# KdaiP/StableTTS

Hardware: NVIDIA H100
Metric: mel-frames/sec through CFM DiT estimator (ODE solve, all evaluations) (higher is better)
Workload: dtype f32 (split-bf16x3 tensor-core operands; FFN convs fp16 activations x fp16 hi/lo weights, 2 passes; fp32 accumulate)

## Files before the change

### stabletts_b200/csrc/gemm_epilogue.cuh

```cuda
#pragma once
#include "common.cuh"
#include <type_traits>
#include "tc_ptx.cuh"

namespace st {

enum : int { EM_PLAIN = 0, EM_SILU = 1, EM_GELU = 2, EM_ROPE = 3, EM_LN = 4, EM_RESID = 5,
             EM_SILU_OUT = 6,
             EM_MISH = 7 };

struct TcParams {
    int n_src, Cs0, Cs1, taps, dil, N, a_bmod, BB, T;
    int m_tiles_per_b, n_tiles, total_tiles;
    int flags, B, film_H, c_clamp, resid_clamp, rope_H;
    long film_bstride, gate_bstride;
    const float *bias, *mask, *film, *gate, *resid, *rope_cs;
    int mode;
    float* out_f32; bf16* out_hi; bf16* out_lo;
    int out16, u16;
    int ln_mask_out;
    const float *ln_shift, *ln_scale, *film2;
    float* out2_f32; bf16* u_hi; bf16* u_lo;
    long ada_bstride, film2_bstride;
    int ksplit, split_bb;
// ... 66 lines not shown

__device__ __forceinline__ float2 lds2_volatile(uint32_t a) {
    float2 v;
    asm volatile("ld.volatile.shared.v2.f32 {%0, %1}, [%2];" : "=f"(v.x), "=f"(v.y) : "r"(a));
    return v;
}

__device__ __forceinline__ void named_bar_sync(int id) { asm volatile("bar.sync %0, 128;" ::"r"(id) : "memory"); }

template <typename T>
__device__ __forceinline__ T* row_ptr(T* base, long off) {
    T* r;
    asm volatile("add.s64 %0, %1, %2;" : "=l"(r) : "l"(base), "l"(off * (long)sizeof(T)));
    return r;
}

__device__ __forceinline__ void st2_if(float* a, float x, float y, bool on) {
    asm volatile("{\n\t.reg .pred q;\n\tsetp.ne.b32 q, %3, 0;\n\t@q st.global.v2.f32 [%0], {%1, %2};\n\t}"
                 ::"l"(a), "f"(x), "f"(y), "r"((int)on));
}
__device__ __forceinline__ void st1_if(bf16* a, uint32_t v, bool on) {
    asm volatile("{\n\t.reg .pred q;\n\tsetp.ne.b32 q, %2, 0;\n\t@q st.global.b32 [%0], %1;\n\t}" ::"l"(a), "r"(v), "r"((int)on));
}

}

enum : int { EV_BIAS = 0, EV_FILM_G, EV_FILM_B, EV_GATE, EV_FILM2_G, EV_FILM2_B, EV_LN_SHIFT, EV_LN_SCALE, EV_COUNT };
constexpr int EPI_VEC_BYTES = EV_COUNT * 256 * 4;

template <int BN, int MODE>
__device__ __forceinline__ void stage_epi_vectors(const TcParams& p, int bb, int n0, uint32_t vs, int bar_id) {
    static_assert(BN == 256, "one column pair per thread of the warpgroup");
    epi::named_bar_sync(bar_id);
    const int c = 2 * (threadIdx.x & 127);
    const int mb = bb % p.B, cb = min(bb, p.c_clamp);
    auto put = [&](int v, const float* src) {
        const float2 x = epi::ld2(src + c);
        asm volatile("st.shared.v2.f32 [%0], {%1, %2};" ::"r"(vs + (v * BN + c) * 4), "f"(x.x), "f"(x.y) : "memory");
    };
    if (p.flags & EPI_BIAS) put(EV_BIAS, p.bias + n0);
    if (MODE != EM_ROPE) {
        if (p.flags & EPI_FILM) {
            const float* film = p.film + (long)mb * p.film_bstride + n0;
            put(EV_FILM_G, film); put(EV_FILM_B, film + p.film_H);
        }
        if (p.flags & EPI_GATE) put(EV_GATE, p.gate + (long)cb * p.gate_bstride + n0);
    }
    if (MODE == EM_LN) {
        const long ab = (long)cb * p.ada_bstride;
        put(EV_LN_SHIFT, p.ln_shift + ab); put(EV_LN_SCALE, p.ln_scale + ab);
        if (p.film2) {
            const float* film2 = p.film2 + (long)mb * p.film2_bstride;
            put(EV_FILM2_G, film2); put(EV_FILM2_B, film2 + p.film_H);
        }
    }
}

template <int MODE>
__device__ __forceinline__ void epilogue_wide(const TcParams& p, int bb, int t0, int n0, float (&acc)[128], uint32_t vs,
                                              int bar_id) {
    using namespace epi;
    constexpr int BN = 256, NJ = BN / 8;
    named_bar_sync(bar_id);
    constexpr bool ROPE = MODE == EM_ROPE, LN = MODE == EM_LN, SO = MODE == EM_SILU_OUT;
    constexpr bool RES = MODE == EM_RESID || MODE == EM_LN || SO;
    const int lane = threadIdx.x & 31, w = (threadIdx.x >> 5) & 3;
    const int cq = 2 * (lane & 3);
    const int mb = bb % p.B;
    const int f = p.flags;
    const bool bias = f & EPI_BIAS, film = f & EPI_FILM, gate = f & EPI_GATE;
    const bool plain = ROPE || (f & (EPI_FILM | EPI_MASK | EPI_GATE | EPI_RESID)) == 0;
    const bool has_resid = RES && (f & EPI_RESID);
    const float rfill = plain || (f & (EPI_FILM | EPI_MASK | EPI_GATE | EPI_RESID)) == EPI_MASK ? -0.f : 0.f;
    const bool f16 = p.out16 != 0, has_film2 = LN && p.film2;
    const bool has_2 = p.out2_f32 && (SO || has_film2);
    const int rope_rot = 2 * p.rope_H - n0, rope_q = p.rope_H - n0;
    constexpr int RD = 8;
    enum : int { FMT_ANY, FMT_F16, FMT_SPLIT };

#pragma unroll
    for (int r = 0; r < 2; ++r) {
        const int t = t0 + 16 * w + (lane >> 2) + 8 * r;
        const bool row_ok = t < p.T;
        const int tcl = min(t, p.T - 1);
        const float mrow = (!ROPE && p.mask) ? __ldg(p.mask + (long)mb * p.T + tcl) : 1.f;
        const float m = (f & EPI_MASK) ? mrow : 1.f;
        const long orow = ((long)bb * p.T + tcl) * p.N + n0 + cq;
        float4 cs4[2];
        if constexpr (ROPE) {
            const float* cs = p.rope_cs + (long)tcl * 32;
            cs4[0] = __ldg(reinterpret_cast<const float4*>(cs + 2 * cq));
            cs4[1] = __ldg(reinterpret_cast<const float4*>(cs + 2 * (8 + cq)));
        }
        const bool st_f32 = row_ok && p.out_f32, st_f16 = row_ok && p.out_hi && f16, st_split = row_ok && p.out_hi && !f16;
        const bool st_2 = row_ok && has_2;
        float* const of = row_ptr(p.out_f32, orow);
        float* const o2 = SO || LN ? row_ptr(p.out2_f32, orow) : nullptr;
        bf16* const oh = row_ptr(p.out_hi, orow);
        bf16* const ol = row_ptr(p.out_lo, orow);
        const float* const rs = RES ? row_ptr(p.resid, ((long)min(bb, p.resid_clamp) * p.T + tcl) * p.N + n0 + cq) : nullptr;
        uint32_t vsr;
        asm volatile("mov.b32 %0, %1;" : "=r"(vsr) : "r"(vs + cq * 4));
        auto vec = [&](int v, int j) { return lds2(vsr + (v * BN + 8 * j) * 4); };
        float s1 = 0.f;

        auto row = [&](auto fmt) {
            float2 ring[RD];
            if constexpr (RES) {
#pragma unroll
                for (int j = 0; j < RD; ++j) ring[j] = ld2_ring(rs + 8 * j, has_resid, rfill);
            }
#pragma unroll
            for (int j = 0; j < NJ; ++j) {
                const int i = (j / 16) * 64 + (j % 16) * 4 + 2 * r;
                float x0 = acc[i], x1 = acc[i + 1];
                float2 rr;
                if constexpr (RES) {
                    rr = ring[j % RD];
                    if (j + RD < NJ) ring[j % RD] = ld2_ring(rs + 8 * (j + RD), has_resid, rfill);
                }
                if constexpr (ROPE) {
                    const int jj = j % 8, hh = j / 8;
                    const bool rot = 64 * hh < rope_rot;
                    if (jj == 0 && rot) {
#pragma unroll
                        for (int k = 0; k < 2; ++k) {
                            const int ia = ((j + k) / 16) * 64 + ((j + k) % 16) * 4 + 2 * r;
                            const int i2 = ((j + k + 2) / 16) * 64 + ((j + k + 2) % 16) * 4 + 2 * r;
                            float u0 = acc[ia], u1 = acc[ia + 1], y0 = acc[i2], y1 = acc[i2 + 1];
                            if (bias) { const float2 b = vec(EV_BIAS, j + k); u0 += b.x; u1 += b.y; }
                            if (bias) { const float2 b = vec(EV_BIAS, j + k + 2); y0 += b.x; y1 += b.y; }
                            const float4 c4 = cs4[k];
                            acc[ia] = u0 * c4.x - y0 * c4.y; acc[ia + 1] = u1 * c4.z - y1 * c4.w;
                            acc[i2] = y0 * c4.x + u0 * c4.y; acc[i2 + 1] = y1 * c4.z + u1 * c4.w;
                        }
                    }
                    x0 = acc[i]; x1 = acc[i + 1];
                    if (bias && !(jj < 4 && rot)) { const float2 b = vec(EV_BIAS, j); x0 += b.x; x1 += b.y; }
                    if (64 * hh < rope_q) { x0 *= kQScale; x1 *= kQScale; }
                } else {
                    float &a0 = acc[i], &a1 = acc[i + 1];
                    if (bias) { const float2 b = vec(EV_BIAS, j); a0 += b.x; a1 += b.y; }
                    if constexpr (MODE == EM_SILU) { a0 = silu_fast(a0); a1 = silu_fast(a1); }
                    if constexpr (MODE == EM_GELU) { a0 = gelu_f(a0); a1 = gelu_f(a1); }
                    if (film) {
                        const float2 fg = vec(EV_FILM_G, j), fb = vec(EV_FILM_B, j);
                        a0 = fmaf(fg.x, a0, fb.x); a1 = fmaf(fg.y, a1, fb.y);
                    }
                    float g0 = m, g1 = m;
                    if (gate) { const float2 g2 = vec(EV_GATE, j); g0 *= g2.x; g1 *= g2.y; }
                    if constexpr (RES) {
                        a0 = fmaf(a0, g0, rr.x); a1 = fmaf(a1, g1, rr.y);
                    } else if (!plain) {
                        a0 *= g0; a1 *= g1;
                    }
                    x0 = a0; x1 = a1;
                }
                st2_if(of + 8 * j, x0, x1, st_f32);
                float h0 = x0, h1 = x1;
                if constexpr (SO) { h0 = silu_fast(x0); h1 = silu_fast(x1); st2_if(o2 + 8 * j, h0, h1, st_2); }
                if constexpr (decltype(fmt)::value != FMT_SPLIT) st1_if(oh + 8 * j, pack_f16x2_sat(h0, h1), st_f16);
                if constexpr (decltype(fmt)::value != FMT_F16) {
                    uint32_t hw, lw;
                    split_bf16x2(h0, h1, hw, lw);
                    st1_if(oh + 8 * j, hw, st_split); st1_if(ol + 8 * j, lw, st_split);
                }
                if constexpr (LN) {
                    if (has_film2) {
                        const float2 fg = vec(EV_FILM2_G, j), fb = vec(EV_FILM2_B, j);
                        x0 = (fg.x * x0 + fb.x) * mrow; x1 = (fg.y * x1 + fb.y) * mrow;
                    }
                    st2_if(o2 + 8 * j, x0, x1, st_2);
                    acc[i] = x0; acc[i + 1] = x1;
                    s1 += x0 + x1;
                }
            }
        };
        if constexpr (RES) {
            row(std::integral_constant<int, FMT_ANY>());
        } else if (f16) {
// ... 22 lines not shown
                const float2 s4 = lds2_volatile(vsr + (EV_LN_SHIFT * BN + 8 * j) * 4);
                const float2 c4 = lds2_volatile(vsr + (EV_LN_SCALE * BN + 8 * j) * 4);
                u0 = ((acc[i] - mean) * rstd * (1.f + c4.x) + s4.x) * mo;
                u1 = ((acc[i + 1] - mean) * rstd * (1.f + c4.y) + s4.y) * mo;
            };
            if (p.u16) {
#pragma unroll
                for (int j = 0; j < NJ; ++j) {
                    float u0, u1;
                    u_pair(j, u0, u1);
                    st1_if(uh + 8 * j, pack_f16x2_sat(u0, u1), row_ok);
                }
            } else {
#pragma unroll
                for (int j = 0; j < NJ; ++j) {
                    float u0, u1;
                    uint32_t hw, lw;
                    u_pair(j, u0, u1);
                    split_bf16x2(u0, u1, hw, lw);
                    st1_if(uh + 8 * j, hw, row_ok); st1_if(ul + 8 * j, lw, row_ok);
                }
            }
        }
    }
}

template <int BN, int MODE>
__device__ __forceinline__ void epilogue_narrow(const TcParams& p, int bb, int t0, int n0, float (&acc)[BN / 2]) {
    using namespace epi;
    constexpr bool ROPE = MODE == EM_ROPE, SO = MODE == EM_SILU_OUT;
    constexpr bool RES = MODE == EM_RESID || SO;
    static_assert(BN <= 128 && MODE != EM_LN, "the fused LayerNorm runs on full-row 256-channel tiles (epilogue_wide)");
    constexpr int NJ = BN / 8;
    const int lane = threadIdx.x & 31, w = (threadIdx.x >> 5) & 3;
    const int cq = 2 * (lane & 3);
    const int mb = bb % p.B;
    const bool plain = ROPE || (p.flags & (EPI_FILM | EPI_MASK | EPI_GATE | EPI_RESID)) == 0;
    const bool mask_only = !ROPE && (p.flags & (EPI_FILM | EPI_MASK | EPI_GATE | EPI_RESID)) == EPI_MASK;
    const bool has_resid = RES && (p.flags & EPI_RESID);
    const float* film = p.film + (long)mb * p.film_bstride;
    const float* gate = p.gate + (long)min(bb, p.c_clamp) * p.gate_bstride;

    constexpr int RD = 8;

#pragma unroll
    for (int r = 0; r < 2; ++r) {
// ... 93 lines not shown
```

### stabletts_b200/csrc/gemm_tc.cu

```cuda
#include "common.cuh"
#include "gemm_epilogue.cuh"
#include <cuda.h>
#include <cudaTypedefs.h>
#include <mutex>
#include <unordered_map>
#include <string>
#include <cstring>
#include <cstdlib>

namespace st {

static_assert(ST_TEST_MODE_PLAIN == EM_PLAIN && ST_TEST_MODE_SILU == EM_SILU && ST_TEST_MODE_GELU == EM_GELU &&
              ST_TEST_MODE_ROPE == EM_ROPE && ST_TEST_MODE_LN == EM_LN && ST_TEST_MODE_RESID == EM_RESID &&
              ST_TEST_MODE_SILU_OUT == EM_SILU_OUT && ST_TEST_MODE_MISH == EM_MISH,
              "st_test_gemm_plan::mode reports the EM_* epilogue instances");

bool tmap_encode_bf16(const void* ptr, int rank, uint64_t d0, uint64_t d1, uint64_t d2, uint32_t b0, uint32_t b1,
                      CUtensorMap* out);

namespace {

using namespace ptx;

constexpr int BLOCK_M = 128;
constexpr int BLOCK_K = 64;
constexpr int WG_K = 16;
constexpr int NUM_THREADS = 384;
constexpr int A_TILE_BYTES = BLOCK_M * BLOCK_K * 2;

struct TcMaps {
    CUtensorMap a_hi[2], a_lo[2], w_hi, w_lo;
};

template <int BN, int PREC> struct Cfg {
    static constexpr int B_TILE_BYTES = BN * BLOCK_K * 2;
    static constexpr int A_BYTES = (PREC ? 1 : 2) * A_TILE_BYTES;
    static constexpr int STAGE_BYTES = A_BYTES + 2 * B_TILE_BYTES;
    static constexpr int STAGES = BN == 256 ? 2 : BN == 128 ? 3 : 4;
    static constexpr int VEC_OFF = STAGES * STAGE_BYTES;
    static constexpr int BAR_OFF = VEC_OFF + (BN == 256 ? 2 * EPI_VEC_BYTES : 0);
    static constexpr int SMEM_BYTES = BAR_OFF + 64  + 1024 ;
    static_assert(SMEM_BYTES <= 227 * 1024, "above the 227 KB of shared memory a block may use on sm_90");
};

template <int BN, int MODE, int PREC>
__global__ void __launch_bounds__(NUM_THREADS, 1)
gemm_wgmma_kernel(const __grid_constant__ TcMaps maps, const TcParams p) {
    using C = Cfg<BN, PREC>;
    extern __shared__ uint8_t smem_raw[];
    uint8_t* smem = reinterpret_cast<uint8_t*>((reinterpret_cast<uintptr_t>(smem_raw) + 1023) & ~uintptr_t(1023));
    uint64_t* full_bar = reinterpret_cast<uint64_t*>(smem + C::BAR_OFF);
    uint64_t* empty_bar = full_bar + C::STAGES;

    pdl_trigger();
    const int wg = threadIdx.x >> 7;
    const int kb0 = (p.Cs0 + BLOCK_K - 1) / BLOCK_K;
    const int kb1 = p.n_src > 1 ? (p.Cs1 + BLOCK_K - 1) / BLOCK_K : 0;
    const int kb_per_tap = kb0 + kb1;
    const int num_kb = p.taps * kb_per_tap;
    const int it_per = (num_kb + p.ksplit - 1) / p.ksplit;
    const int pad = p.taps / 2;

    if (threadIdx.x == 0) {
        prefetch_tmap(&maps.a_hi[0]); prefetch_tmap(&maps.a_lo[0]); prefetch_tmap(&maps.w_hi); prefetch_tmap(&maps.w_lo);
        if (p.n_src > 1) { prefetch_tmap(&maps.a_hi[1]); prefetch_tmap(&maps.a_lo[1]); }
        for (int i = 0; i < C::STAGES; ++i) { mbar_init(&full_bar[i], 1); mbar_init(&empty_bar[i], 8); }
        mbar_fence_init();
    }
    __syncthreads();
    pdl_wait();

    if (wg == 0) {
        reg_dealloc<40>();
        if (threadIdx.x == 0) {
            int stage = 0; uint32_t phase = 0;
            for (int tile = blockIdx.x; tile < p.total_tiles; tile += gridDim.x) {
                const int n_tile = tile % p.n_tiles, m_tile = tile / p.n_tiles;
                const int bb = m_tile / p.m_tiles_per_b, t0 = (m_tile % p.m_tiles_per_b) * BLOCK_M;
                const int ab = (bb % p.split_bb) % p.a_bmod, n0 = n_tile * BN;
                const int it0 = (bb / p.split_bb) * it_per, it1 = min(num_kb, it0 + it_per);
                for (int it = it0; it < it1; ++it) {
                    const int kb = it / p.taps, tap = it % p.taps;
                    const int src = kb >= kb0 ? 1 : 0;
                    const int kc = (src ? kb - kb0 : kb) * BLOCK_K;
                    const int kw = (src ? p.Cs0 : 0) + kc;
                    mbar_wait(&empty_bar[stage], phase ^ 1);
                    uint8_t* s = smem + stage * C::STAGE_BYTES;
                    mbar_expect_tx(&full_bar[stage], C::STAGE_BYTES);
                    const int ta = t0 + (tap - pad) * p.dil;
                    tma_load_3d(&maps.a_hi[src], &full_bar[stage], s, kc, ta, ab);
                    if (!PREC) tma_load_3d(&maps.a_lo[src], &full_bar[stage], s + A_TILE_BYTES, kc, ta, ab);
                    tma_load_2d(&maps.w_hi, &full_bar[stage], s + C::A_BYTES, kw, tap * p.N + n0);
                    tma_load_2d(&maps.w_lo, &full_bar[stage], s + C::A_BYTES + C::B_TILE_BYTES, kw, tap * p.N + n0);
                    if (++stage == C::STAGES) { stage = 0; phase ^= 1; }
                }
            }
        }
    } else {
        reg_alloc<232>();
        const int cw = wg - 1;
        float acc[BN / 2];
        int stage = 0; uint32_t phase = 0;
        for (int tile = blockIdx.x; tile < p.total_tiles; tile += gridDim.x) {
            const int n_tile = tile % p.n_tiles, m_tile = tile / p.n_tiles;
            const int bb = m_tile / p.m_tiles_per_b, t0 = (m_tile % p.m_tiles_per_b) * BLOCK_M + cw * 64;
            const uint32_t vs = smem_u32(smem + C::VEC_OFF + cw * EPI_VEC_BYTES);
            if constexpr (BN == 256) stage_epi_vectors<BN, MODE>(p, bb, n_tile * BN, vs, 1 + cw);
            const int it0 = (bb / p.split_bb) * it_per;
            const int n_it = min(num_kb, it0 + it_per) - it0;
            for (int kb = 0; kb < n_it; ++kb) {
                mbar_wait(&full_bar[stage], phase);
                const uint32_t sa = smem_u32(smem + stage * C::STAGE_BYTES) + (uint32_t)cw * (64 * 128);
                const uint32_t sb = smem_u32(smem + stage * C::STAGE_BYTES) + C::A_BYTES;
                const uint64_t a_hi = make_sw128_desc(sa), a_lo = make_sw128_desc(sa + A_TILE_BYTES);
                wgmma_fence();
#pragma unroll
                for (int k = 0; k < BLOCK_K / WG_K; ++k) {
                    const uint64_t adv = (uint64_t)((k * WG_K * 2) >> 4);
                    if constexpr (BN < 128) {
                        const uint64_t b_hi = make_sw128_desc(sb) + adv, b_lo = make_sw128_desc(sb + C::B_TILE_BYTES) + adv;
                        const int acc_in = (kb | k) != 0;
                        if constexpr (BN == 64) {
                            wgmma_m64n64k16_ss(acc, a_lo + adv, b_hi, acc_in);
                            wgmma_m64n64k16_ss(acc, a_hi + adv, b_lo, 1);
                            wgmma_m64n64k16_ss(acc, a_hi + adv, b_hi, 1);
                        } else if constexpr (BN == 32) {
                            wgmma_m64n32k16_ss(acc, a_lo + adv, b_hi, acc_in);
                            wgmma_m64n32k16_ss(acc, a_hi + adv, b_lo, 1);
                            wgmma_m64n32k16_ss(acc, a_hi + adv, b_hi, 1);
                        } else {
                            wgmma_m64n16k16_ss(acc, a_lo + adv, b_hi, acc_in);
                            wgmma_m64n16k16_ss(acc, a_hi + adv, b_lo, 1);
                            wgmma_m64n16k16_ss(acc, a_hi + adv, b_hi, 1);
                        }
                    }
#pragma unroll
                    for (int h = 0; h < BN / 128; ++h) {
                        float (&d)[64] = *reinterpret_cast<float (*)[64]>(&acc[64 * h]);
                        const uint64_t b_hi = make_sw128_desc(sb + h * (128 * 128)) + adv;
                        const uint64_t b_lo = make_sw128_desc(sb + C::B_TILE_BYTES + h * (128 * 128)) + adv;
                        if (PREC) {
                            wgmma_m64n128k16_ss<true>(d, a_hi + adv, b_lo, (kb | k) != 0);
                            wgmma_m64n128k16_ss<true>(d, a_hi + adv, b_hi, 1);
                        } else {
                            wgmma_m64n128k16_ss<false>(d, a_lo + adv, b_hi, (kb | k) != 0);
                            wgmma_m64n128k16_ss<false>(d, a_hi + adv, b_lo, 1);
                            wgmma_m64n128k16_ss<false>(d, a_hi + adv, b_hi, 1);
                        }
                    }
                }
                wgmma_commit();
                wgmma_wait<0>();
                if ((threadIdx.x & 31) == 0) mbar_arrive(&empty_bar[stage]);
                if (++stage == C::STAGES) { stage = 0; phase ^= 1; }
            }
            epilogue_tile<BN, MODE>(p, bb, t0, n_tile * BN, acc, vs, 1 + cw);
        }
    }
}

std::string g_err = "";
std::recursive_mutex g_mu;
PFN_cuTensorMapEncodeTiled_v12000 g_encode = nullptr;

struct MapKey {
    const void* ptr; uint64_t d0, d1, d2; uint32_t b0, b1; int rank;
    bool operator==(const MapKey& o) const {
        return ptr == o.ptr && d0 == o.d0 && d1 == o.d1 && d2 == o.d2 && b0 == o.b0 && b1 == o.b1 && rank == o.rank;
    }
};
struct MapKeyHash {
    size_t operator()(const MapKey& k) const {
        size_t h = std::hash<const void*>()(k.ptr);
        h ^= k.d0 * 0x9E3779B97F4A7C15ull + (h << 6); h ^= k.d1 * 0xC2B2AE3D27D4EB4Full + (h >> 3);
        h ^= k.d2 * 0x165667B19E3779F9ull + (h << 9); h ^= ((size_t)k.b0 << 20) ^ ((size_t)k.b1 << 4) ^ (size_t)k.rank;
        return h;
    }
};
std::unordered_map<MapKey, CUtensorMap, MapKeyHash> g_maps;
// ... 19 lines not shown
    const uint64_t es = 2;
    cuuint64_t dims[3] = {d0, d1, d2};
    cuuint64_t strides[2] = {d0 * es, d0 * d1 * es};
    cuuint32_t box[3] = {b0, b1, 1};
    cuuint32_t estr[3] = {1, 1, 1};
    CUtensorMap m;
    CUresult r = g_encode(&m, CU_TENSOR_MAP_DATA_TYPE_BFLOAT16, (cuuint32_t)rank,
                          const_cast<void*>(ptr), dims, strides, box, estr, CU_TENSOR_MAP_INTERLEAVE_NONE,
                          CU_TENSOR_MAP_SWIZZLE_128B, CU_TENSOR_MAP_L2_PROMOTION_L2_256B,
                          CU_TENSOR_MAP_FLOAT_OOB_FILL_NONE);
    if (r != CUDA_SUCCESS) {
        g_err = "cuTensorMapEncodeTiled failed with CUresult " + std::to_string((int)r) + " (rank " + std::to_string(rank) +
                ", dims " + std::to_string(d0) + "x" + std::to_string(d1) + "x" + std::to_string(d2) + ")";
        return false;
    }
    if (g_maps.size() > 4096) g_maps.clear();
    g_maps.emplace(key, m);
    *out = m;
    return true;
}

template <int BN, int MODE, int PREC>
cudaError_t launch_inst(const TcMaps& maps, const TcParams& p, int grid, cudaStream_t s) {
    using C = Cfg<BN, PREC>;
    static std::atomic<uint64_t> attr_done{0};
    cudaError_t e = ensure_dyn_smem(gemm_wgmma_kernel<BN, MODE, PREC>, C::SMEM_BYTES, attr_done);
    if (e != cudaSuccess) { g_err = "cudaFuncSetAttribute(max dynamic smem) failed"; return e; }
    g_inst.engine = ST_ENGINE_TCGEN05; g_inst.bn = BN; g_inst.mode = MODE; g_inst.prec = PREC; g_inst.ksplit = p.ksplit; g_inst.grid = grid;
    return launch_k(gemm_wgmma_kernel<BN, MODE, PREC>, dim3(grid), dim3(NUM_THREADS), (size_t)C::SMEM_BYTES, s, maps, p);
}

template <int BN>
cudaError_t launch_bn(const GemmArgs& g, int num_sms, cudaStream_t s, int split_bb = 0) {
    TcMaps maps;
    for (int i = 0; i < g.n_src; ++i) {
        if (!tmap_encode_bf16(g.A_hi[i], 3, (uint64_t)g.Cs[i], (uint64_t)g.T, (uint64_t)g.a_bmod, BLOCK_K, BLOCK_M, &maps.a_hi[i])) return cudaErrorInvalidValue;
        if (g.prec) maps.a_lo[i] = maps.a_hi[i];
        else if (!tmap_encode_bf16(g.A_lo[i], 3, (uint64_t)g.Cs[i], (uint64_t)g.T, (uint64_t)g.a_bmod, BLOCK_K, BLOCK_M, &maps.a_lo[i])) return cudaErrorInvalidValue;
    }
    if (g.n_src == 1) { maps.a_hi[1] = maps.a_hi[0]; maps.a_lo[1] = maps.a_lo[0]; }
    if (!tmap_encode_bf16(g.W_hi, 2, (uint64_t)g.Ktot, (uint64_t)g.taps * g.N, 1, BLOCK_K, BN, &maps.w_hi)) return cudaErrorInvalidValue;
    if (!tmap_encode_bf16(g.W_lo, 2, (uint64_t)g.Ktot, (uint64_t)g.taps * g.N, 1, BLOCK_K, BN, &maps.w_lo)) return cudaErrorInvalidValue;
    TcParams p;
    fill_tc_params(p, g);
    if (split_bb > 0) { p.ksplit = g.ksplit; p.split_bb = split_bb; }
    p.m_tiles_per_b = (g.T + BLOCK_M - 1) / BLOCK_M;
    p.n_tiles = (g.N + BN - 1) / BN;
    p.total_tiles = g.BB * p.m_tiles_per_b * p.n_tiles;
    const int grid = p.total_tiles < num_sms ? p.total_tiles : num_sms;
    if (p.mode == EM_MISH) {
        if constexpr (BN == 128) return launch_inst<BN, EM_MISH, 0>(maps, p, grid, s);
        g_err = "EPI_MISH runs on 128-channel tiles only"; return cudaErrorInvalidValue;
    }
    if constexpr (BN == 256) {
        if (g.N % 256) { g_err = "256-channel tiles need N % 256 == 0"; return cudaErrorInvalidValue; }
        if ((g.flags & EPI_ROPE) && g.rope_H % 64) { g_err = "RoPE on 256-channel tiles needs rope_H % 64 == 0"; return cudaErrorInvalidValue; }
        if (g.prec) {
            switch (p.mode) {
                case EM_SILU:  return launch_inst<BN, EM_SILU, 1>(maps, p, grid, s);
                case EM_LN:    return launch_inst<BN, EM_LN, 1>(maps, p, grid, s);
                case EM_RESID: return launch_inst<BN, EM_RESID, 1>(maps, p, grid, s);
                case EM_PLAIN: return launch_inst<BN, EM_PLAIN, 1>(maps, p, grid, s);
                default: g_err = "the two-pass fp16 precision is built for the FFN and long-skip convs only"; return cudaErrorInvalidValue;
            }
        }
// ... 12 lines not shown
    switch (p.mode) {
        case EM_ROPE: return launch_inst<BN, EM_ROPE, 0>(maps, p, grid, s);
        case EM_SILU: return launch_inst<BN, EM_SILU, 0>(maps, p, grid, s);
        case EM_GELU: return launch_inst<BN, EM_GELU, 0>(maps, p, grid, s);
        case EM_RESID: return launch_inst<BN, EM_RESID, 0>(maps, p, grid, s);
        case EM_SILU_OUT: return launch_inst<BN, EM_SILU_OUT, 0>(maps, p, grid, s);
        default:      return launch_inst<BN, EM_PLAIN, 0>(maps, p, grid, s);
    }
}

}

const char* gemm_tc_last_error() { return g_err.c_str(); }

bool tmap_encode_bf16(const void* ptr, int rank, uint64_t d0, uint64_t d1, uint64_t d2, uint32_t b0, uint32_t b1,
                      CUtensorMap* out) {
    std::lock_guard<std::recursive_mutex> lk(g_mu);
    if (!ensure_encode()) return false;
    return get_map(ptr, rank, d0, d1, d2, b0, b1, out);
}

static bool wide_tile(const GemmArgs& g, int num_sms) {
    if (!g.A_hi[0] || !g.W_hi || g.N % 256 || (g.flags & EPI_MISH)) return false;
    return (long)g.BB * ((g.T + BLOCK_M - 1) / BLOCK_M) * (g.N / 256) >= num_sms;
}

bool gemm_tc_wide_tile(const GemmArgs& g, int num_sms) { return wide_tile(g, num_sms); }

bool gemm_tc_ln_fusable(const GemmArgs& g, int num_sms) { return g.N == 256 && wide_tile(g, num_sms); }

static cudaError_t launch_gemm_tc_locked(const GemmArgs& g, int num_sms, cudaStream_t s);

cudaError_t launch_gemm_tc(const GemmArgs& g, int num_sms, cudaStream_t s) {
    if (g.BB == 0 || g.T == 0) return cudaSuccess;
    std::lock_guard<std::recursive_mutex> lk(g_mu);
    g_inst = GemmPlan();
    const cudaError_t e = launch_gemm_tc_locked(g, num_sms, s);
    if (e == cudaSuccess && g.plan) *g.plan = g_inst;
    return e;
}

static cudaError_t launch_gemm_tc_locked(const GemmArgs& g, int num_sms, cudaStream_t s) {
    if (const char* why = gemm_flags_error(g)) { g_err = why; return cudaErrorInvalidValue; }
    const bool wide = wide_tile(g, num_sms);
    if (g.dil < 1) { g_err = "tap dilation must be >= 1"; return cudaErrorInvalidValue; }
    if (g.ln && g.N != 256) {
// ... 50 lines not shown
```

Baseline: 305,900.

## Add dedicated RoPE QKV GEMM path with resident A slab and 128-wide half tiles

```diff
diff --git a/stabletts_b200/csrc/gemm_epilogue.cuh b/stabletts_b200/csrc/gemm_epilogue.cuh
--- a/stabletts_b200/csrc/gemm_epilogue.cuh
+++ b/stabletts_b200/csrc/gemm_epilogue.cuh
@@ -112,6 +112,10 @@
 __device__ __forceinline__ void st1_if(bf16* a, uint32_t v, bool on) {
     asm volatile("{\n\t.reg .pred q;\n\tsetp.ne.b32 q, %2, 0;\n\t@q st.global.b32 [%0], %1;\n\t}" ::"l"(a), "r"(v), "r"((int)on));
 }
+__device__ __forceinline__ void st2w_if(bf16* a, uint32_t v0, uint32_t v1, bool on) {
+    asm volatile("{\n\t.reg .pred q;\n\tsetp.ne.b32 q, %3, 0;\n\t@q st.global.v2.b32 [%0], {%1, %2};\n\t}"
+                 ::"l"(a), "r"(v0), "r"(v1), "r"((int)on));
+}
 
 }
 
@@ -120,7 +124,7 @@
 
 template <int BN, int MODE>
 __device__ __forceinline__ void stage_epi_vectors(const TcParams& p, int bb, int n0, uint32_t vs, int bar_id) {
-    static_assert(BN == 256, "one column pair per thread of the warpgroup");
+    static_assert(BN == 256 && MODE != EM_ROPE, "one column pair per thread of the warpgroup (RoPE: stage_rope_bias)");
     epi::named_bar_sync(bar_id);
     const int c = 2 * (threadIdx.x & 127);
     const int mb = bb % p.B, cb = min(bb, p.c_clamp);
@@ -129,13 +133,11 @@
         asm volatile("st.shared.v2.f32 [%0], {%1, %2};" ::"r"(vs + (v * BN + c) * 4), "f"(x.x), "f"(x.y) : "memory");
     };
     if (p.flags & EPI_BIAS) put(EV_BIAS, p.bias + n0);
-    if (MODE != EM_ROPE) {
-        if (p.flags & EPI_FILM) {
-            const float* film = p.film + (long)mb * p.film_bstride + n0;
-            put(EV_FILM_G, film); put(EV_FILM_B, film + p.film_H);
-        }
-        if (p.flags & EPI_GATE) put(EV_GATE, p.gate + (long)cb * p.gate_bstride + n0);
-    }
+    if (p.flags & EPI_FILM) {
+        const float* film = p.film + (long)mb * p.film_bstride + n0;
+        put(EV_FILM_G, film); put(EV_FILM_B, film + p.film_H);
+    }
+    if (p.flags & EPI_GATE) put(EV_GATE, p.gate + (long)cb * p.gate_bstride + n0);
     if (MODE == EM_LN) {
         const long ab = (long)cb * p.ada_bstride;
         put(EV_LN_SHIFT, p.ln_shift + ab); put(EV_LN_SCALE, p.ln_scale + ab);
@@ -150,21 +152,21 @@
 __device__ __forceinline__ void epilogue_wide(const TcParams& p, int bb, int t0, int n0, float (&acc)[128], uint32_t vs,
                                               int bar_id) {
     using namespace epi;
+    static_assert(MODE != EM_ROPE, "RoPE: epilogue_rope_half");
     constexpr int BN = 256, NJ = BN / 8;
     named_bar_sync(bar_id);
-    constexpr bool ROPE = MODE == EM_ROPE, LN = MODE == EM_LN, SO = MODE == EM_SILU_OUT;
+    constexpr bool LN = MODE == EM_LN, SO = MODE == EM_SILU_OUT;
     constexpr bool RES = MODE == EM_RESID || MODE == EM_LN || SO;
     const int lane = threadIdx.x & 31, w = (threadIdx.x >> 5) & 3;
     const int cq = 2 * (lane & 3);
     const int mb = bb % p.B;
     const int f = p.flags;
     const bool bias = f & EPI_BIAS, film = f & EPI_FILM, gate = f & EPI_GATE;
-    const bool plain = ROPE || (f & (EPI_FILM | EPI_MASK | EPI_GATE | EPI_RESID)) == 0;
+    const bool plain = (f & (EPI_FILM | EPI_MASK | EPI_GATE | EPI_RESID)) == 0;
     const bool has_resid = RES && (f & EPI_RESID);
     const float rfill = plain || (f & (EPI_FILM | EPI_MASK | EPI_GATE | EPI_RESID)) == EPI_MASK ? -0.f : 0.f;
     const bool f16 = p.out16 != 0, has_film2 = LN && p.film2;
     const bool has_2 = p.out2_f32 && (SO || has_film2);
-    const int rope_rot = 2 * p.rope_H - n0, rope_q = p.rope_H - n0;
     constexpr int RD = 8;
     enum : int { FMT_ANY, FMT_F16, FMT_SPLIT };
 
@@ -173,15 +175,9 @@
         const int t = t0 + 16 * w + (lane >> 2) + 8 * r;
         const bool row_ok = t < p.T;
         const int tcl = min(t, p.T - 1);
-        const float mrow = (!ROPE && p.mask) ? __ldg(p.mask + (long)mb * p.T + tcl) : 1.f;
+        const float mrow = p.mask ? __ldg(p.mask + (long)mb * p.T + tcl) : 1.f;
         const float m = (f & EPI_MASK) ? mrow : 1.f;
         const long orow = ((long)bb * p.T + tcl) * p.N + n0 + cq;
-        float4 cs4[2];
-        if constexpr (ROPE) {
-            const float* cs = p.rope_cs + (long)tcl * 32;
-            cs4[0] = __ldg(reinterpret_cast<const float4*>(cs + 2 * cq));
-            cs4[1] = __ldg(reinterpret_cast<const float4*>(cs + 2 * (8 + cq)));
-        }
         const bool st_f32 = row_ok && p.out_f32, st_f16 = row_ok && p.out_hi && f16, st_split = row_ok && p.out_hi && !f16;
         const bool st_2 = row_ok && has_2;
         float* const of = row_ptr(p.out_f32, orow);
@@ -203,49 +199,27 @@
 #pragma unroll
             for (int j = 0; j < NJ; ++j) {
                 const int i = (j / 16) * 64 + (j % 16) * 4 + 2 * r;
-                float x0 = acc[i], x1 = acc[i + 1];
                 float2 rr;
                 if constexpr (RES) {
                     rr = ring[j % RD];
                     if (j + RD < NJ) ring[j % RD] = ld2_ring(rs + 8 * (j + RD), has_resid, rfill);
                 }
-                if constexpr (ROPE) {
-                    const int jj = j % 8, hh = j / 8;
-                    const bool rot = 64 * hh < rope_rot;
-                    if (jj == 0 && rot) {
-#pragma unroll
-                        for (int k = 0; k < 2; ++k) {
-                            const int ia = ((j + k) / 16) * 64 + ((j + k) % 16) * 4 + 2 * r;
-                            const int i2 = ((j + k + 2) / 16) * 64 + ((j + k + 2) % 16) * 4 + 2 * r;
-                            float u0 = acc[ia], u1 = acc[ia + 1], y0 = acc[i2], y1 = acc[i2 + 1];
-                            if (bias) { const float2 b = vec(EV_BIAS, j + k); u0 += b.x; u1 += b.y; }
-                            if (bias) { const float2 b = vec(EV_BIAS, j + k + 2); y0 += b.x; y1 += b.y; }
-                            const float4 c4 = cs4[k];
-                            acc[ia] = u0 * c4.x - y0 * c4.y; acc[ia + 1] = u1 * c4.z - y1 * c4.w;
-                            acc[i2] = y0 * c4.x + u0 * c4.y; acc[i2 + 1] = y1 * c4.z + u1 * c4.w;
-                        }
-                    }
-                    x0 = acc[i]; x1 = acc[i + 1];
-                    if (bias && !(jj < 4 && rot)) { const float2 b = vec(EV_BIAS, j); x0 += b.x; x1 += b.y; }
-                    if (64 * hh < rope_q) { x0 *= kQScale; x1 *= kQScale; }
-                } else {
-                    float &a0 = acc[i], &a1 = acc[i + 1];
-                    if (bias) { const float2 b = vec(EV_BIAS, j); a0 += b.x; a1 += b.y; }
-                    if constexpr (MODE == EM_SILU) { a0 = silu_fast(a0); a1 = silu_fast(a1); }
-                    if constexpr (MODE == EM_GELU) { a0 = gelu_f(a0); a1 = gelu_f(a1); }
-                    if (film) {
-                        const float2 fg = vec(EV_FILM_G, j), fb = vec(EV_FILM_B, j);
-                        a0 = fmaf(fg.x, a0, fb.x); a1 = fmaf(fg.y, a1, fb.y);
-                    }
-                    float g0 = m, g1 = m;
-                    if (gate) { const float2 g2 = vec(EV_GATE, j); g0 *= g2.x; g1 *= g2.y; }
-                    if constexpr (RES) {
-                        a0 = fmaf(a0, g0, rr.x); a1 = fmaf(a1, g1, rr.y);
-                    } else if (!plain) {
-                        a0 *= g0; a1 *= g1;
-                    }
-                    x0 = a0; x1 = a1;
-                }
+                float &a0 = acc[i], &a1 = acc[i + 1];
+                if (bias) { const float2 b = vec(EV_BIAS, j); a0 += b.x; a1 += b.y; }
+                if constexpr (MODE == EM_SILU) { a0 = silu_fast(a0); a1 = silu_fast(a1); }
+                if constexpr (MODE == EM_GELU) { a0 = gelu_f(a0); a1 = gelu_f(a1); }
+                if (film) {
+                    const float2 fg = vec(EV_FILM_G, j), fb = vec(EV_FILM_B, j);
+                    a0 = fmaf(fg.x, a0, fb.x); a1 = fmaf(fg.y, a1, fb.y);
+                }
+                float g0 = m, g1 = m;
+                if (gate) { const float2 g2 = vec(EV_GATE, j); g0 *= g2.x; g1 *= g2.y; }
+                if constexpr (RES) {
+                    a0 = fmaf(a0, g0, rr.x); a1 = fmaf(a1, g1, rr.y);
+                } else if (!plain) {
+                    a0 *= g0; a1 *= g1;
+                }
+                float x0 = a0, x1 = a1;
                 st2_if(of + 8 * j, x0, x1, st_f32);
                 float h0 = x0, h1 = x1;
                 if constexpr (SO) { h0 = silu_fast(x0); h1 = silu_fast(x1); st2_if(o2 + 8 * j, h0, h1, st_2); }
@@ -314,6 +288,104 @@
                 }
             }
         }
+    }
+}
+
+__device__ __forceinline__ void stage_rope_bias(const TcParams& p, int n0, uint32_t vs, int bar_id) {
+    epi::named_bar_sync(bar_id);
+    if (p.flags & EPI_BIAS) {
+        const int c = threadIdx.x & 127;
+        asm volatile("st.shared.f32 [%0], %1;" ::"r"(vs + 4 * c), "f"(__ldg(p.bias + n0 + c)) : "memory");
+    }
+}
+
+__device__ __forceinline__ void epilogue_rope_half(const TcParams& p, int bb, int t0, int n0, float (&acc)[128], uint32_t vs,
+                                                   int bar_id) {
+    using namespace epi;
+    constexpr int NJ = 128 / 8;
+    named_bar_sync(bar_id);
+    const int lane = threadIdx.x & 31, w = (threadIdx.x >> 5) & 3;
+    const int cq = 2 * (lane & 3);
+    const bool odd = lane & 1;
+    const bool bias = p.flags & EPI_BIAS, f16 = p.out16 != 0;
+    const int rope_rot = 2 * p.rope_H - n0, rope_q = p.rope_H - n0;
+    enum : int { FMT_F16, FMT_SPLIT };
+
+#pragma unroll 1
+    for (int rh = 0; rh < 2; ++rh) {
+        int tcl2[2];
+#pragma unroll
+        for (int r = 0; r < 2; ++r) {
+            const int tc = min(t0 + 64 * rh + 16 * w + (lane >> 2) + 8 * r, p.T - 1);
+            asm volatile("mov.b32 %0, %1;" : "=r"(tcl2[r]) : "r"(tc));
+        }
+#pragma unroll
+        for (int r = 0; r < 2; ++r) {
+            const int t = t0 + 64 * rh + 16 * w + (lane >> 2) + 8 * r;
+            const bool row_ok = t < p.T;
+            const int tcl = tcl2[r];
+            const long orow = ((long)bb * p.T + tcl) * p.N + n0 + cq;
+            const float* cs = p.rope_cs + (long)tcl * 32;
+            const float4 cs4[2] = {__ldg(reinterpret_cast<const float4*>(cs + 2 * cq)),
+                                   __ldg(reinterpret_cast<const float4*>(cs + 2 * (8 + cq)))};
+            const bool st_f32 = row_ok && p.out_f32, st_f16 = row_ok && p.out_hi && f16, st_split = row_ok && p.out_hi && !f16;
+            float* const of = row_ptr(p.out_f32, orow);
+            bf16* const oh = row_ptr(p.out_hi, orow + (odd ? 6 : 0));
+            bf16* const ol = row_ptr(p.out_lo, orow + (odd ? 6 : 0));
+            uint32_t vsr;
+            asm volatile("mov.b32 %0, %1;" : "=r"(vsr) : "r"(vs + cq * 4));
+            auto vec = [&](int j) { return lds2(vsr + 8 * j * 4); };
+            auto st_pair = [&](bf16* o, int j, uint32_t w0, uint32_t w1, bool on) {
+                const uint32_t got = __shfl_xor_sync(0xffffffffu, odd ? w0 : w1, 1);
+                st2w_if(o + 8 * j, odd ? got : w0, odd ? w1 : got, on);
+            };
+
+            auto row = [&](auto fmt) {
+                uint32_t wh = 0, wl = 0;
+#pragma unroll
+                for (int j = 0; j < NJ; ++j) {
+                    const int i = 4 * j + 2 * r;
+                    const int jj = j % 8, hh = j / 8;
+                    const bool rot = 64 * hh < rope_rot;
+                    if (jj == 0 && rot) {
+#pragma unroll
+                        for (int k = 0; k < 2; ++k) {
+                            const int ia = 4 * (j + k) + 2 * r, i2 = 4 * (j + k + 2) + 2 * r;
+                            float u0 = acc[ia], u1 = acc[ia + 1], y0 = acc[i2], y1 = acc[i2 + 1];
+                            if (bias) { const float2 b = vec(j + k); u0 += b.x; u1 += b.y; }
+                            if (bias) { const float2 b = vec(j + k + 2); y0 += b.x; y1 += b.y; }
+                            const float4 c4 = cs4[k];
+                            acc[ia] = u0 * c4.x - y0 * c4.y; acc[ia + 1] = u1 * c4.z - y1 * c4.w;
+                            acc[i2] = y0 * c4.x + u0 * c4.y; acc[i2 + 1] = y1 * c4.z + u1 * c4.w;
+                        }
+                    }
+                    float x0 = acc[i], x1 = acc[i + 1];
+                    if (bias && !(jj < 4 && rot)) { const float2 b = vec(j); x0 += b.x; x1 += b.y; }
+                    if (64 * hh < rope_q) { x0 *= kQScale; x1 *= kQScale; }
+                    st2_if(of + 8 * j, x0, x1, st_f32);
+                    uint32_t hw, lw = 0;
+                    if constexpr (decltype(fmt)::value == FMT_F16) {
+                        hw = pack_f16x2_sat(x0, x1);
+                    } else {
+                        split_bf16x2(x0, x1, hw, lw);
+                    }
+                    if (j % 2 == 0) {
+                        wh = hw; wl = lw;
+                    } else if constexpr (decltype(fmt)::value == FMT_F16) {
+                        st_pair(oh, j - 1, wh, hw, st_f16);
+                    } else {
+                        st_pair(oh, j - 1, wh, hw, st_split); st_pair(ol, j - 1, wl, lw, st_split);
+                    }
+                }
+            };
+            if (f16) {
+                row(std::integral_constant<int, FMT_F16>());
+            } else {
+                row(std::integral_constant<int, FMT_SPLIT>());
+            }
+        }
+#pragma unroll
+        for (int i = 0; i < 64; ++i) acc[i] = acc[64 + i];
     }
 }
 
diff --git a/stabletts_b200/csrc/gemm_tc.cu b/stabletts_b200/csrc/gemm_tc.cu
--- a/stabletts_b200/csrc/gemm_tc.cu
+++ b/stabletts_b200/csrc/gemm_tc.cu
@@ -43,28 +43,47 @@
     static_assert(SMEM_BYTES <= 227 * 1024, "above the 227 KB of shared memory a block may use on sm_90");
 };
 
-template <int BN, int MODE, int PREC>
-__global__ void __launch_bounds__(NUM_THREADS, 1)
-gemm_wgmma_kernel(const __grid_constant__ TcMaps maps, const TcParams p) {
-    using C = Cfg<BN, PREC>;
-    extern __shared__ uint8_t smem_raw[];
-    uint8_t* smem = reinterpret_cast<uint8_t*>((reinterpret_cast<uintptr_t>(smem_raw) + 1023) & ~uintptr_t(1023));
+struct RopeCfg {
+    static constexpr int SLAB_KB = 4;
+    static constexpr int KB_BYTES = 2 * A_TILE_BYTES;
+    static constexpr int W_TILE_BYTES = 128 * BLOCK_K * 2;
+    static constexpr int STAGE_BYTES = 2 * W_TILE_BYTES;
+    static constexpr int STAGES = 3;
+    static constexpr int RING_OFF = SLAB_KB * KB_BYTES;
+    static constexpr int VEC_OFF = RING_OFF + STAGES * STAGE_BYTES;
+    static constexpr int BAR_OFF = VEC_OFF + 2 * 128 * 4;
+    static constexpr int SMEM_BYTES = BAR_OFF + 2 * (STAGES + SLAB_KB) * 8 + 1024 ;
+    static_assert(SMEM_BYTES <= 227 * 1024, "above the 227 KB of shared memory a block may use on sm_90");
+};
+
+template <int BN, int MODE, int PREC> constexpr bool kRopeTiles = BN == 256 && MODE == EM_ROPE && PREC == 0;
+template <int BN, int MODE, int PREC> constexpr int kSmemBytes = kRopeTiles<BN, MODE, PREC> ? RopeCfg::SMEM_BYTES : Cfg<BN, PREC>::SMEM_BYTES;
+
+constexpr int ORDER_BAR = 3;
+
+__device__ __forceinline__ void bar_arrive_n(int id, int n) { asm volatile("bar.arrive %0, %1;" ::"r"(id), "r"(n) : "memory"); }
+__device__ __forceinline__ void bar_sync_n(int id, int n) { asm volatile("bar.sync %0, %1;" ::"r"(id), "r"(n) : "memory"); }
+
+__device__ __forceinline__ void rope_tiles(const TcMaps& maps, const TcParams& p, uint8_t* smem) {
+    using C = RopeCfg;
     uint64_t* full_bar = reinterpret_cast<uint64_t*>(smem + C::BAR_OFF);
     uint64_t* empty_bar = full_bar + C::STAGES;
-
-    pdl_trigger();
+    uint64_t* a_full = empty_bar + C::STAGES;
+    uint64_t* a_empty = a_full + C::SLAB_KB;
     const int wg = threadIdx.x >> 7;
     const int kb0 = (p.Cs0 + BLOCK_K - 1) / BLOCK_K;
     const int kb1 = p.n_src > 1 ? (p.Cs1 + BLOCK_K - 1) / BLOCK_K : 0;
-    const int kb_per_tap = kb0 + kb1;
-    const int num_kb = p.taps * kb_per_tap;
-    const int it_per = (num_kb + p.ksplit - 1) / p.ksplit;
+    const int num_kb = p.taps * (kb0 + kb1);
     const int pad = p.taps / 2;
+    const int hpb = 2 * p.n_tiles;
+    const int h_begin = 2 * (int)((long)blockIdx.x * p.total_tiles / gridDim.x);
+    const int h_end = 2 * (int)((long)(blockIdx.x + 1) * p.total_tiles / gridDim.x);
 
     if (threadIdx.x == 0) {
         prefetch_tmap(&maps.a_hi[0]); prefetch_tmap(&maps.a_lo[0]); prefetch_tmap(&maps.w_hi); prefetch_tmap(&maps.w_lo);
         if (p.n_src > 1) { prefetch_tmap(&maps.a_hi[1]); prefetch_tmap(&maps.a_lo[1]); }
-        for (int i = 0; i < C::STAGES; ++i) { mbar_init(&full_bar[i], 1); mbar_init(&empty_bar[i], 8); }
+        for (int i = 0; i < C::STAGES; ++i) { mbar_init(&full_bar[i], 1); mbar_init(&empty_bar[i], 4); }
+        for (int i = 0; i < C::SLAB_KB; ++i) { mbar_init(&a_full[i], 1); mbar_init(&a_empty[i], 8); }
         mbar_fence_init();
     }
     __syncthreads();
@@ -73,88 +92,206 @@
     if (wg == 0) {
         reg_dealloc<40>();
         if (threadIdx.x == 0) {
-            int stage = 0; uint32_t phase = 0;
-            for (int tile = blockIdx.x; tile < p.total_tiles; tile += gridDim.x) {
-                const int n_tile = tile % p.n_tiles, m_tile = tile / p.n_tiles;
+            int stage = 0, slab = -1; uint32_t phase = 0, a_phase = 0;
+            for (int h = h_begin; h < h_end; ++h) {
+                const int m_tile = h / hpb, n0 = (h % hpb) * 128;
                 const int bb = m_tile / p.m_tiles_per_b, t0 = (m_tile % p.m_tiles_per_b) * BLOCK_M;
-                const int ab = (bb % p.split_bb) % p.a_bmod, n0 = n_tile * BN;
-                const int it0 = (bb / p.split_bb) * it_per, it1 = min(num_kb, it0 + it_per);
-                for (int it = it0; it < it1; ++it) {
+                const bool load_a = m_tile != slab;
+                for (int it = 0; it < num_kb; ++it) {
                     const int kb = it / p.taps, tap = it % p.taps;
                     const int src = kb >= kb0 ? 1 : 0;
                     const int kc = (src ? kb - kb0 : kb) * BLOCK_K;
                     const int kw = (src ? p.Cs0 : 0) + kc;
+                    if (load_a) {
+                        mbar_wait(&a_empty[it], a_phase ^ 1);
+                        uint8_t* s = smem + it * C::KB_BYTES;
+                        mbar_expect_tx(&a_full[it], C::KB_BYTES);
+                        const int ta = t0 + (tap - pad) * p.dil;
+                        tma_load_3d(&maps.a_hi[src], &a_full[it], s, kc, ta, bb % p.a_bmod);
+                        tma_load_3d(&maps.a_lo[src], &a_full[it], s + A_TILE_BYTES, kc, ta, bb % p.a_bmod);
+                    }
                     mbar_wait(&empty_bar[stage], phase ^ 1);
-                    uint8_t* s = smem + stage * C::STAGE_BYTES;
+                    uint8_t* s = smem + C::RING_OFF + stage * C::STAGE_BYTES;
                     mbar_expect_tx(&full_bar[stage], C::STAGE_BYTES);
-                    const int ta = t0 + (tap - pad) * p.dil;
-                    tma_load_3d(&maps.a_hi[src], &full_bar[stage], s, kc, ta, ab);
-                    if (!PREC) tma_load_3d(&maps.a_lo[src], &full_bar[stage], s + A_TILE_BYTES, kc, ta, ab);
-                    tma_load_2d(&maps.w_hi, &full_bar[stage], s + C::A_BYTES, kw, tap * p.N + n0);
-                    tma_load_2d(&maps.w_lo, &full_bar[stage], s + C::A_BYTES + C::B_TILE_BYTES, kw, tap * p.N + n0);
+                    tma_load_2d(&maps.w_hi, &full_bar[stage], s, kw, tap * p.N + n0);
+                    tma_load_2d(&maps.w_lo, &full_bar[stage], s + C::W_TILE_BYTES, kw, tap * p.N + n0);
                     if (++stage == C::STAGES) { stage = 0; phase ^= 1; }
                 }
+                if (load_a) { slab = m_tile; a_phase ^= 1; }
             }
         }
     } else {
         reg_alloc<232>();
         const int cw = wg - 1;
-        float acc[BN / 2];
-        int stage = 0; uint32_t phase = 0;
-        for (int tile = blockIdx.x; tile < p.total_tiles; tile += gridDim.x) {
-            const int n_tile = tile % p.n_tiles, m_tile = tile / p.n_tiles;
-            const int bb = m_tile / p.m_tiles_per_b, t0 = (m_tile % p.m_tiles_per_b) * BLOCK_M + cw * 64;
-            const uint32_t vs = smem_u32(smem + C::VEC_OFF + cw * EPI_VEC_BYTES);
-            if constexpr (BN == 256) stage_epi_vectors<BN, MODE>(p, bb, n_tile * BN, vs, 1 + cw);
-            const int it0 = (bb / p.split_bb) * it_per;
-            const int n_it = min(num_kb, it0 + it_per) - it0;
-            for (int kb = 0; kb < n_it; ++kb) {
+        const uint32_t vs = smem_u32(smem + C::VEC_OFF + cw * 128 * 4);
+        float acc[128];
+        int slab = -1; uint32_t a_phase = 0;
+        for (int h = h_begin + cw; h < h_end; h += 2) {
+            const int m_tile = h / hpb, n0 = (h % hpb) * 128;
+            const int bb = m_tile / p.m_tiles_per_b, t0 = (m_tile % p.m_tiles_per_b) * BLOCK_M;
+            if (m_tile != slab) { a_phase ^= slab >= 0; slab = m_tile; }
+            const bool last_of_slab = h + 2 >= h_end || (h + 2) / hpb != m_tile;
+            stage_rope_bias(p, n0, vs, 1 + cw);
+            const int pos = (h - h_begin) * num_kb;
+            int stage = pos % C::STAGES, prev = 0;
+            uint32_t phase = (pos / C::STAGES) & 1;
+            if (h > h_begin) bar_sync_n(ORDER_BAR + cw, 256);
+            for (int it = 0; it < num_kb; ++it) {
+                mbar_wait(&a_full[it], a_phase);
                 mbar_wait(&full_bar[stage], phase);
-                const uint32_t sa = smem_u32(smem + stage * C::STAGE_BYTES) + (uint32_t)cw * (64 * 128);
-                const uint32_t sb = smem_u32(smem + stage * C::STAGE_BYTES) + C::A_BYTES;
-                const uint64_t a_hi = make_sw128_desc(sa), a_lo = make_sw128_desc(sa + A_TILE_BYTES);
+                const uint32_t sa = smem_u32(smem + it * C::KB_BYTES);
+                const uint32_t sb = smem_u32(smem + C::RING_OFF + stage * C::STAGE_BYTES);
                 wgmma_fence();
 #pragma unroll
                 for (int k = 0; k < BLOCK_K / WG_K; ++k) {
                     const uint64_t adv = (uint64_t)((k * WG_K * 2) >> 4);
-                    if constexpr (BN < 128) {
-                        const uint64_t b_hi = make_sw128_desc(sb) + adv, b_lo = make_sw128_desc(sb + C::B_TILE_BYTES) + adv;
-                        const int acc_in = (kb | k) != 0;
-                        if constexpr (BN == 64) {
-                            wgmma_m64n64k16_ss(acc, a_lo + adv, b_hi, acc_in);
-                            wgmma_m64n64k16_ss(acc, a_hi + adv, b_lo, 1);
-                            wgmma_m64n64k16_ss(acc, a_hi + adv, b_hi, 1);
-                        } else if constexpr (BN == 32) {
-                            wgmma_m64n32k16_ss(acc, a_lo + adv, b_hi, acc_in);
-                            wgmma_m64n32k16_ss(acc, a_hi + adv, b_lo, 1);
-                            wgmma_m64n32k16_ss(acc, a_hi + adv, b_hi, 1);
-                        } else {
-                            wgmma_m64n16k16_ss(acc, a_lo + adv, b_hi, acc_in);
-                            wgmma_m64n16k16_ss(acc, a_hi + adv, b_lo, 1);
-                            wgmma_m64n16k16_ss(acc, a_hi + adv, b_hi, 1);
-                        }
-                    }
+                    const uint64_t b_hi = make_sw128_desc(sb) + adv, b_lo = make_sw128_desc(sb + C::W_TILE_BYTES) + adv;
 #pragma unroll
-                    for (int h = 0; h < BN / 128; ++h) {
-                        float (&d)[64] = *reinterpret_cast<float (*)[64]>(&acc[64 * h]);
-                        const uint64_t b_hi = make_sw128_desc(sb + h * (128 * 128)) + adv;
-                        const uint64_t b_lo = make_sw128_desc(sb + C::B_TILE_BYTES + h * (128 * 128)) + adv;
-                        if (PREC) {
-                            wgmma_m64n128k16_ss<true>(d, a_hi + adv, b_lo, (kb | k) != 0);
-                            wgmma_m64n128k16_ss<true>(d, a_hi + adv, b_hi, 1);
-                        } else {
-                            wgmma_m64n128k16_ss<false>(d, a_lo + adv, b_hi, (kb | k) != 0);
-                            wgmma_m64n128k16_ss<false>(d, a_hi + adv, b_lo, 1);
-                            wgmma_m64n128k16_ss<false>(d, a_hi + adv, b_hi, 1);
-                        }
+                    for (int rh = 0; rh < 2; ++rh) {
+                        float (&d)[64] = *reinterpret_cast<float (*)[64]>(&acc[64 * rh]);
+                        const uint64_t a_hi = make_sw128_desc(sa + rh * (64 * 128)) + adv;
+                        const uint64_t a_lo = make_sw128_desc(sa + A_TILE_BYTES + rh * (64 * 128)) + adv;
+                        wgmma_m64n128k16_ss<false>(d, a_lo, b_hi, (it | k) != 0);
+                        wgmma_m64n128k16_ss<false>(d, a_hi, b_lo, 1);
+                        wgmma_m64n128k16_ss<false>(d, a_hi, b_hi, 1);
                     }
                 }
                 wgmma_commit();
-                wgmma_wait<0>();
-                if ((threadIdx.x & 31) == 0) mbar_arrive(&empty_bar[stage]);
+                wgmma_wait<1>();
+                if (it > 0 && (threadIdx.x & 31) == 0) {
+                    mbar_arrive(&empty_bar[prev]);
+                    if (last_of_slab) mbar_arrive(&a_empty[it - 1]);
+                }
+                prev = stage;
                 if (++stage == C::STAGES) { stage = 0; phase ^= 1; }
             }
-            epilogue_tile<BN, MODE>(p, bb, t0, n_tile * BN, acc, vs, 1 + cw);
+            if (h + 1 < h_end) bar_arrive_n(ORDER_BAR + 1 - cw, 256);
+            wgmma_wait<0>();
+            if ((threadIdx.x & 31) == 0) {
+                mbar_arrive(&empty_bar[prev]);
+                if (last_of_slab) mbar_arrive(&a_empty[num_kb - 1]);
+            }
+            epilogue_rope_half(p, bb, t0, n0, acc, vs, 1 + cw);
+        }
+    }
+}
+
+template <int BN, int MODE, int PREC>
+__global__ void __launch_bounds__(NUM_THREADS, 1)
+gemm_wgmma_kernel(const __grid_constant__ TcMaps maps, const TcParams p) {
+    extern __shared__ uint8_t smem_raw[];
+    uint8_t* smem = reinterpret_cast<uint8_t*>((reinterpret_cast<uintptr_t>(smem_raw) + 1023) & ~uintptr_t(1023));
+    pdl_trigger();
+    if constexpr (kRopeTiles<BN, MODE, PREC>) {
+        rope_tiles(maps, p, smem);
+    } else {
+        using C = Cfg<BN, PREC>;
+        uint64_t* full_bar = reinterpret_cast<uint64_t*>(smem + C::BAR_OFF);
+        uint64_t* empty_bar = full_bar + C::STAGES;
+
+        const int wg = threadIdx.x >> 7;
+        const int kb0 = (p.Cs0 + BLOCK_K - 1) / BLOCK_K;
+        const int kb1 = p.n_src > 1 ? (p.Cs1 + BLOCK_K - 1) / BLOCK_K : 0;
+        const int kb_per_tap = kb0 + kb1;
+        const int num_kb = p.taps * kb_per_tap;
+        const int it_per = (num_kb + p.ksplit - 1) / p.ksplit;
+        const int pad = p.taps / 2;
+
+        if (threadIdx.x == 0) {
+            prefetch_tmap(&maps.a_hi[0]); prefetch_tmap(&maps.a_lo[0]); prefetch_tmap(&maps.w_hi); prefetch_tmap(&maps.w_lo);
+            if (p.n_src > 1) { prefetch_tmap(&maps.a_hi[1]); prefetch_tmap(&maps.a_lo[1]); }
+            for (int i = 0; i < C::STAGES; ++i) { mbar_init(&full_bar[i], 1); mbar_init(&empty_bar[i], 8); }
+            mbar_fence_init();
+        }
+        __syncthreads();
+        pdl_wait();
+
+        if (wg == 0) {
+            reg_dealloc<40>();
+            if (threadIdx.x == 0) {
+                int stage = 0; uint32_t phase = 0;
+                for (int tile = blockIdx.x; tile < p.total_tiles; tile += gridDim.x) {
+                    const int n_tile = tile % p.n_tiles, m_tile = tile / p.n_tiles;
+                    const int bb = m_tile / p.m_tiles_per_b, t0 = (m_tile % p.m_tiles_per_b) * BLOCK_M;
+                    const int ab = (bb % p.split_bb) % p.a_bmod, n0 = n_tile * BN;
+                    const int it0 = (bb / p.split_bb) * it_per, it1 = min(num_kb, it0 + it_per);
+                    for (int it = it0; it < it1; ++it) {
+                        const int kb = it / p.taps, tap = it % p.taps;
+                        const int src = kb >= kb0 ? 1 : 0;
+                        const int kc = (src ? kb - kb0 : kb) * BLOCK_K;
+                        const int kw = (src ? p.Cs0 : 0) + kc;
+                        mbar_wait(&empty_bar[stage], phase ^ 1);
+                        uint8_t* s = smem + stage * C::STAGE_BYTES;
+                        mbar_expect_tx(&full_bar[stage], C::STAGE_BYTES);
+                        const int ta = t0 + (tap - pad) * p.dil;
+                        tma_load_3d(&maps.a_hi[src], &full_bar[stage], s, kc, ta, ab);
+                        if (!PREC) tma_load_3d(&maps.a_lo[src], &full_bar[stage], s + A_TILE_BYTES, kc, ta, ab);
+                        tma_load_2d(&maps.w_hi, &full_bar[stage], s + C::A_BYTES, kw, tap * p.N + n0);
+                        tma_load_2d(&maps.w_lo, &full_bar[stage], s + C::A_BYTES + C::B_TILE_BYTES, kw, tap * p.N + n0);
+                        if (++stage == C::STAGES) { stage = 0; phase ^= 1; }
+                    }
+                }
+            }
+        } else {
+            reg_alloc<232>();
+            const int cw = wg - 1;
+            float acc[BN / 2];
+            int stage = 0; uint32_t phase = 0;
+            for (int tile = blockIdx.x; tile < p.total_tiles; tile += gridDim.x) {
+                const int n_tile = tile % p.n_tiles, m_tile = tile / p.n_tiles;
+                const int bb = m_tile / p.m_tiles_per_b, t0 = (m_tile % p.m_tiles_per_b) * BLOCK_M + cw * 64;
+                const uint32_t vs = smem_u32(smem + C::VEC_OFF + cw * EPI_VEC_BYTES);
+                if constexpr (BN == 256) stage_epi_vectors<BN, MODE>(p, bb, n_tile * BN, vs, 1 + cw);
+                const int it0 = (bb / p.split_bb) * it_per;
+                const int n_it = min(num_kb, it0 + it_per) - it0;
+                for (int kb = 0; kb < n_it; ++kb) {
+                    mbar_wait(&full_bar[stage], phase);
+                    const uint32_t sa = smem_u32(smem + stage * C::STAGE_BYTES) + (uint32_t)cw * (64 * 128);
+                    const uint32_t sb = smem_u32(smem + stage * C::STAGE_BYTES) + C::A_BYTES;
+                    const uint64_t a_hi = make_sw128_desc(sa), a_lo = make_sw128_desc(sa + A_TILE_BYTES);
+                    wgmma_fence();
+    #pragma unroll
+                    for (int k = 0; k < BLOCK_K / WG_K; ++k) {
+                        const uint64_t adv = (uint64_t)((k * WG_K * 2) >> 4);
+                        if constexpr (BN < 128) {
+                            const uint64_t b_hi = make_sw128_desc(sb) + adv, b_lo = make_sw128_desc(sb + C::B_TILE_BYTES) + adv;
+                            const int acc_in = (kb | k) != 0;
+                            if constexpr (BN == 64) {
+                                wgmma_m64n64k16_ss(acc, a_lo + adv, b_hi, acc_in);
+                                wgmma_m64n64k16_ss(acc, a_hi + adv, b_lo, 1);
+                                wgmma_m64n64k16_ss(acc, a_hi + adv, b_hi, 1);
+                            } else if constexpr (BN == 32) {
+                                wgmma_m64n32k16_ss(acc, a_lo + adv, b_hi, acc_in);
+                                wgmma_m64n32k16_ss(acc, a_hi + adv, b_lo, 1);
+                                wgmma_m64n32k16_ss(acc, a_hi + adv, b_hi, 1);
+                            } else {
+                                wgmma_m64n16k16_ss(acc, a_lo + adv, b_hi, acc_in);
+                                wgmma_m64n16k16_ss(acc, a_hi + adv, b_lo, 1);
+                                wgmma_m64n16k16_ss(acc, a_hi + adv, b_hi, 1);
+                            }
+                        }
+    #pragma unroll
+                        for (int h = 0; h < BN / 128; ++h) {
+                            float (&d)[64] = *reinterpret_cast<float (*)[64]>(&acc[64 * h]);
+                            const uint64_t b_hi = make_sw128_desc(sb + h * (128 * 128)) + adv;
+                            const uint64_t b_lo = make_sw128_desc(sb + C::B_TILE_BYTES + h * (128 * 128)) + adv;
+                            if (PREC) {
+                                wgmma_m64n128k16_ss<true>(d, a_hi + adv, b_lo, (kb | k) != 0);
+                                wgmma_m64n128k16_ss<true>(d, a_hi + adv, b_hi, 1);
+                            } else {
+                                wgmma_m64n128k16_ss<false>(d, a_lo + adv, b_hi, (kb | k) != 0);
+                                wgmma_m64n128k16_ss<false>(d, a_hi + adv, b_lo, 1);
+                                wgmma_m64n128k16_ss<false>(d, a_hi + adv, b_hi, 1);
+                            }
+                        }
+                    }
+                    wgmma_commit();
+                    wgmma_wait<0>();
+                    if ((threadIdx.x & 31) == 0) mbar_arrive(&empty_bar[stage]);
+                    if (++stage == C::STAGES) { stage = 0; phase ^= 1; }
+                }
+                epilogue_tile<BN, MODE>(p, bb, t0, n_tile * BN, acc, vs, 1 + cw);
+            }
         }
     }
 }
@@ -220,12 +357,12 @@
 
 template <int BN, int MODE, int PREC>
 cudaError_t launch_inst(const TcMaps& maps, const TcParams& p, int grid, cudaStream_t s) {
-    using C = Cfg<BN, PREC>;
+    constexpr int SMEM = kSmemBytes<BN, MODE, PREC>;
     static std::atomic<uint64_t> attr_done{0};
-    cudaError_t e = ensure_dyn_smem(gemm_wgmma_kernel<BN, MODE, PREC>, C::SMEM_BYTES, attr_done);
+    cudaError_t e = ensure_dyn_smem(gemm_wgmma_kernel<BN, MODE, PREC>, SMEM, attr_done);
     if (e != cudaSuccess) { g_err = "cudaFuncSetAttribute(max dynamic smem) failed"; return e; }
     g_inst.engine = ST_ENGINE_TCGEN05; g_inst.bn = BN; g_inst.mode = MODE; g_inst.prec = PREC; g_inst.ksplit = p.ksplit; g_inst.grid = grid;
-    return launch_k(gemm_wgmma_kernel<BN, MODE, PREC>, dim3(grid), dim3(NUM_THREADS), (size_t)C::SMEM_BYTES, s, maps, p);
+    return launch_k(gemm_wgmma_kernel<BN, MODE, PREC>, dim3(grid), dim3(NUM_THREADS), (size_t)SMEM, s, maps, p);
 }
 
 template <int BN>
@@ -237,8 +374,9 @@
         else if (!tmap_encode_bf16(g.A_lo[i], 3, (uint64_t)g.Cs[i], (uint64_t)g.T, (uint64_t)g.a_bmod, BLOCK_K, BLOCK_M, &maps.a_lo[i])) return cudaErrorInvalidValue;
     }
     if (g.n_src == 1) { maps.a_hi[1] = maps.a_hi[0]; maps.a_lo[1] = maps.a_lo[0]; }
-    if (!tmap_encode_bf16(g.W_hi, 2, (uint64_t)g.Ktot, (uint64_t)g.taps * g.N, 1, BLOCK_K, BN, &maps.w_hi)) return cudaErrorInvalidValue;
-    if (!tmap_encode_bf16(g.W_lo, 2, (uint64_t)g.Ktot, (uint64_t)g.taps * g.N, 1, BLOCK_K, BN, &maps.w_lo)) return cudaErrorInvalidValue;
+    const uint32_t wrows = BN == 256 && (g.flags & EPI_ROPE) ? 128 : BN;
+    if (!tmap_encode_bf16(g.W_hi, 2, (uint64_t)g.Ktot, (uint64_t)g.taps * g.N, 1, BLOCK_K, wrows, &maps.w_hi)) return cudaErrorInvalidValue;
+    if (!tmap_encode_bf16(g.W_lo, 2, (uint64_t)g.Ktot, (uint64_t)g.taps * g.N, 1, BLOCK_K, wrows, &maps.w_lo)) return cudaErrorInvalidValue;
     TcParams p;
     fill_tc_params(p, g);
     if (split_bb > 0) { p.ksplit = g.ksplit; p.split_bb = split_bb; }
@@ -297,6 +435,8 @@
 
 static bool wide_tile(const GemmArgs& g, int num_sms) {
     if (!g.A_hi[0] || !g.W_hi || g.N % 256 || (g.flags & EPI_MISH)) return false;
+    const int kblocks = (g.Cs[0] + BLOCK_K - 1) / BLOCK_K + (g.n_src > 1 ? (g.Cs[1] + BLOCK_K - 1) / BLOCK_K : 0);
+    if ((g.flags & EPI_ROPE) && g.taps * kblocks > RopeCfg::SLAB_KB) return false;
     return (long)g.BB * ((g.T + BLOCK_M - 1) / BLOCK_M) * (g.N / 256) >= num_sms;
 }
 
```

Result: faster. 321,300, median of 6 (+5.0%).
